# ipc-sim/IPC

Measured on NVIDIA H100. Metric: newton_iteration_ms_assembly_ccd, lower is better.
Workload: dtype f64

## Files before the change

ipc_b200/csrc/api.cu:

```cuda
#include "../../include/ipcgpu.h"
#include "context.h"
#include <algorithm>
#include <cmath>
#include <cstring>
#include <dlfcn.h>
#include <numeric>

using namespace ipcgpu;

#define CK(call)                                                                                  \
    do {                                                                                          \
        cudaError_t e_ = (call);                                                                  \
        if (e_ != cudaSuccess) {                                                                  \
            ctx->err = std::string(#call) + ": " + cudaGetErrorString(e_);                        \
            return IPCGPU_ERR_CUDA;                                                               \
        }                                                                                         \
    } while (0)
#define REQUIRE(cond, code, msg)                                                                  \
    do {                                                                                          \
        if (!(cond)) {                                                                            \
            ctx->err = (msg);                                                                     \
            return (code);                                                                        \
        }                                                                                         \
    } while (0)
// ... 16 lines not shown
bool nccl_load(std::string& err)
{
    if (g_nccl.h) return true;
    const char* names[] = { "libnccl.so.2", "libnccl.so" };
    for (const char* n : names) {
        g_nccl.h = dlopen(n, RTLD_NOW | RTLD_GLOBAL);
        if (g_nccl.h) break;
    }
    if (!g_nccl.h) {
        err = "dlopen(libnccl.so.2) failed";
        return false;
    }
    g_nccl.GetUniqueId = (int (*)(void*))dlsym(g_nccl.h, "ncclGetUniqueId");
    g_nccl.CommInitRank = (int (*)(void**, int, Id128, int))dlsym(g_nccl.h, "ncclCommInitRank");
    g_nccl.AllReduce = (int (*)(const void*, void*, size_t, int, int, void*, cudaStream_t))dlsym(g_nccl.h, "ncclAllReduce");
    g_nccl.AllGather = (int (*)(const void*, void*, size_t, int, void*, cudaStream_t))dlsym(g_nccl.h, "ncclAllGather");
    g_nccl.CommDestroy = (int (*)(void*))dlsym(g_nccl.h, "ncclCommDestroy");
    g_nccl.GetErrorString = (const char* (*)(int))dlsym(g_nccl.h, "ncclGetErrorString");
    if (!g_nccl.GetUniqueId || !g_nccl.CommInitRank || !g_nccl.AllReduce || !g_nccl.AllGather) {
        err = "NCCL symbols missing";
        return false;
    }
    return true;
}
constexpr int kNcclInt32 = 2;
constexpr int kNcclFloat64 = 8;
constexpr int kNcclUint64 = 5;
constexpr int kNcclSum = 0, kNcclMax = 2, kNcclMin = 3;
}

int nccl_min_u64(ipcgpu_ctx* ctx, unsigned long long* word)
{
    if (ctx->nranks <= 1) return IPCGPU_OK;
    cudaEvent_t pe = ctx->prof_begin(IPCGPU_STAGE_ALLREDUCE);
    int r = g_nccl.AllReduce(word, word, 1, kNcclUint64, kNcclMin, ctx->nccl_comm, ctx->stream);
    ctx->prof_end(pe);
    REQUIRE(r == 0, IPCGPU_ERR_NCCL, "ncclAllReduce(min step) failed");
    return IPCGPU_OK;
}

static int join_copy_stream(ipcgpu_ctx* ctx)
{
    if (!ctx->copy_pending) return IPCGPU_OK;
    CK(cudaEventRecord(ctx->ev_copy_join, ctx->copy));
    CK(cudaStreamWaitEvent(ctx->stream, ctx->ev_copy_join, 0));
    ctx->copy_pending = false;
    return IPCGPU_OK;
}

enum Chain { kSerial, kStepBound, kDerivative };

static int join_deriv(ipcgpu_ctx* ctx)
{
    if (!ctx->deriv_open) return IPCGPU_OK;
    ctx->deriv_open = false;
    CK(cudaEventRecord(ctx->ev_deriv_done, ctx->deriv));
    CK(cudaStreamWaitEvent(ctx->stream, ctx->ev_deriv_done, 0));
    return IPCGPU_OK;
}

static int enter(ipcgpu_ctx* ctx, Chain chain)
{
    if (chain == kStepBound) return IPCGPU_OK;
    if (chain == kSerial || ctx->nranks > 1 || ctx->profiling) return join_deriv(ctx);
    if (ctx->deriv_open) return IPCGPU_OK;
    CK(cudaEventRecord(ctx->ev_deriv_fork, ctx->stream));
    CK(cudaStreamWaitEvent(ctx->deriv, ctx->ev_deriv_fork, 0));
    ctx->deriv_open = true;
    return IPCGPU_OK;
}
#define ENTER(chain)                                                                              \
    do {                                                                                          \
        int re_ = enter(ctx, (chain));                                                            \
        if (re_) return re_;                                                                      \
    } while (0)

int fetch_iter_state(ipcgpu_ctx* ctx)
{
    {
        int rcj = join_copy_stream(ctx);
        if (rcj) return rcj;
    }
    CK(cudaMemcpyAsync(ctx->h_iter, ctx->iter.p, sizeof(IterState), cudaMemcpyDeviceToHost, ctx->stream));
    CK(cudaStreamSynchronize(ctx->stream));
    return IPCGPU_OK;
}
static int clear_flag(ipcgpu_ctx* ctx, int idx)
{
    CK(cudaMemsetAsync(&ctx->iter.p->flags[idx], 0, sizeof(int), ctx->stream));
    return IPCGPU_OK;
}

static int build_maps(ipcgpu_ctx* ctx)
{
    const int nT = ctx->nT, nV = ctx->nV;
    const std::vector<int>& T = ctx->h_T;
    ctx->t_begin = (int)((int64_t)nT * ctx->rank / ctx->nranks);
    ctx->t_end = (int)((int64_t)nT * (ctx->rank + 1) / ctx->nranks);
    std::vector<int64_t> cum(nV + 1, 0);
    for (size_t i = 0; i < (size_t)4 * nT; ++i) ++cum[T[i] + 1];
    for (int v = 0; v < nV; ++v) cum[v + 1] += cum[v];
    auto boundary = [&](int r) -> int {
        if (r <= 0) return 0;
        if (r >= ctx->nranks) return nV;
        const int64_t target = cum[nV] * r / ctx->nranks;
        return (int)(std::lower_bound(cum.begin(), cum.end(), target) - cum.begin());
// ... 1099 lines not shown
int ipcgpu_update_pattern(ipcgpu_ctx* ctx, int with_friction, int* changed, int64_t* nnz)
{
    REQUIRE(ctx->device_pattern, IPCGPU_ERR_STATE, "ipcgpu_enable_device_pattern first");
    REQUIRE(ctx->surface_ready, IPCGPU_ERR_STATE, "ipcgpu_set_surface first");
    REQUIRE(!with_friction || ctx->cw.fr_ready, IPCGPU_ERR_STATE, "with_friction: ipcgpu_friction_lag / ipcgpu_set_friction_data first");
    CK(cudaSetDevice(ctx->device));
    ENTER(kSerial);
    int rc = pattern_update(ctx, barrier_args(ctx, 1.0, 1.0, 0), with_friction != 0);
    if (rc) return rc;
    ctx->pat_pending = true;
    if (!changed && !nnz) return IPCGPU_OK;
    if ((rc = sync_pattern_mirror(ctx))) return rc;
    if (changed) *changed = ctx->pat_changed_host;
    if (nnz) *nnz = ctx->nnz;
    if (ctx->h_iter->flags[FLAG_PATTERN_CAPACITY]) {
        clear_flag(ctx, FLAG_PATTERN_CAPACITY);
        int only[8] = { 0 };
        only[FLAG_PATTERN_CAPACITY] = 1;
        return status_from_flags(ctx, only);
    }
    return IPCGPU_OK;
}

int ipcgpu_pattern_info(ipcgpu_ctx* ctx, int* changed, int64_t* nnz, uint64_t* version)
{
    REQUIRE(ctx->device_pattern, IPCGPU_ERR_STATE, "ipcgpu_enable_device_pattern first");
    CK(cudaSetDevice(ctx->device));
    ENTER(kSerial);
    int rc = sync_pattern_mirror(ctx);
    if (rc) return rc;
    if (changed) *changed = ctx->pat_changed_host;
    if (nnz) *nnz = ctx->nnz;
    if (version) *version = ctx->pat_seen_version;
    return IPCGPU_OK;
}

int ipcgpu_get_pattern(ipcgpu_ctx* ctx, int* ia, int* ja)
{
    REQUIRE(ctx->n_rows > 0, IPCGPU_ERR_STATE, "no pattern: ipcgpu_set_csr or ipcgpu_enable_device_pattern first");
    CK(cudaSetDevice(ctx->device));
    ENTER(kSerial);
    int rc = sync_pattern_mirror(ctx);
    if (rc) return rc;
    if (ia) CK(cudaMemcpyAsync(ia, ctx->ia.p, ((size_t)ctx->n_rows + 1) * sizeof(int), cudaMemcpyDeviceToHost, ctx->stream));
    if (ja) CK(cudaMemcpyAsync(ja, ctx->ja.p, (size_t)ctx->nnz * sizeof(int), cudaMemcpyDeviceToHost, ctx->stream));
    CK(cudaStreamSynchronize(ctx->stream));
    return IPCGPU_OK;
}

int ipcgpu_barrier_energy(ipcgpu_ctx* ctx, double dHat, double kappa, double* E)
{
    REQUIRE(ctx->surface_ready, IPCGPU_ERR_STATE, "ipcgpu_set_surface first");
    CK(cudaSetDevice(ctx->device));
    ENTER(kSerial);
    BarrierArgs p = barrier_args(ctx, dHat, kappa, 0);
    cudaEvent_t pe = ctx->prof_begin(IPCGPU_STAGE_BARRIER);
    barrier_energy(p, ctx->cw.bpartials.p, &ctx->iter.p->flags[FLAG_NONPOSITIVE_DISTANCE], ctx->stream);
    reduce_sum(ctx->cw.bpartials.p, barrier_energy_blocks(), kappa, ctx->scalar_out.p + 1, ctx->stream);
    ctx->prof_end(pe);
    ctx->launches += 2;
    if (ctx->nranks > 1 && E) {
        int r = g_nccl.AllReduce(ctx->scalar_out.p + 1, ctx->scalar_out.p + 1, 1, kNcclFloat64, kNcclSum, ctx->nccl_comm, ctx->stream);
        REQUIRE(r == 0, IPCGPU_ERR_NCCL, "ncclAllReduce(barrier energy) failed");
    }
    energy_store(ctx->iter.p, 1, ctx->scalar_out.p + 1, ctx->stream);
    ++ctx->launches;
    ctx->energy_local[1] = (ctx->nranks > 1 && !E);
    CK(cudaGetLastError());
    if (E) {
        int rc = fetch_iter_state(ctx);
        if (rc) return rc;
        *E = ctx->h_iter->energy[1];
        if (ctx->h_iter->flags[FLAG_NONPOSITIVE_DISTANCE]) {
            clear_flag(ctx, FLAG_NONPOSITIVE_DISTANCE);
            int only[8] = { 0 };
            only[FLAG_NONPOSITIVE_DISTANCE] = 1;
            return status_from_flags(ctx, only);
        }
    }
    return IPCGPU_OK;
}

int ipcgpu_barrier_gradient(ipcgpu_ctx* ctx, double dHat, double kappa, double* g_inout)
{
    REQUIRE(ctx->surface_ready, IPCGPU_ERR_STATE, "ipcgpu_set_surface first");
    CK(cudaSetDevice(ctx->device));
    ENTER(g_inout ? kSerial : kDerivative);
    if (g_inout) {
        if (ctx->rank == 0) CK(cudaMemcpyAsync(ctx->g.p, g_inout, (size_t)3 * ctx->nV * sizeof(double), cudaMemcpyHostToDevice, ctx->stream));
        else CK(cudaMemsetAsync(ctx->g.p, 0, (size_t)3 * ctx->nV * sizeof(double), ctx->stream));
    }
    cudaEvent_t pe = ctx->prof_begin(IPCGPU_STAGE_BARRIER);
    barrier_gradient(barrier_args(ctx, dHat, kappa, 0), ctx->g.p, ctx->deriv_stream());
    ctx->prof_end(pe);
    ++ctx->launches;
    CK(cudaGetLastError());
    if (g_inout && ctx->nranks > 1) {
        int rc = ipcgpu_allreduce_grad_hess(ctx, 1, 0);
        if (rc) return rc;
    }
    if (g_inout) {
        CK(cudaMemcpyAsync(g_inout, ctx->g.p, (size_t)3 * ctx->nV * sizeof(double), cudaMemcpyDeviceToHost, ctx->stream));
        CK(cudaStreamSynchronize(ctx->stream));
    }
    return IPCGPU_OK;
}

static int gradient_roundtrip_begin(ipcgpu_ctx* ctx, const double* g_in)
{
    if (ctx->rank == 0) CK(cudaMemcpyAsync(ctx->g.p, g_in, (size_t)3 * ctx->nV * sizeof(double), cudaMemcpyHostToDevice, ctx->stream));
    else CK(cudaMemsetAsync(ctx->g.p, 0, (size_t)3 * ctx->nV * sizeof(double), ctx->stream));
    return IPCGPU_OK;
}
static int gradient_roundtrip_end(ipcgpu_ctx* ctx, double* g_out)
{
    if (ctx->nranks > 1) {
        int rc = ipcgpu_allreduce_grad_hess(ctx, 1, 0);
        if (rc) return rc;
// ... 32 lines not shown
    CK(cudaSetDevice(ctx->device));
    ENTER(kSerial);
    ContactWork& w = ctx->cw;
    if (w.nC < 0) {
        int rc = contact_sync_counts(ctx);
        if (rc) return rc;
    }
    REQUIRE(n == w.nC && (input || n == 0), IPCGPU_ERR_ARG, "ipcgpu_constraint_jacobian_t: n must be the size of the active set on this context");
    REQUIRE(!(ctx->nranks > 1 && ctx->lists_local), IPCGPU_ERR_STATE, "per-constraint input needs the replicated sets (ipcgpu_set_contact_partition(0))");
    ALLOC(w.bval, (size_t)std::max(w.cap, 1));
    int rc = gradient_roundtrip_begin(ctx, g_inout);
    if (rc) return rc;
    if (n) CK(cudaMemcpyAsync(w.bval.p, input, (size_t)n * sizeof(double), cudaMemcpyHostToDevice, ctx->stream));
    BarrierArgs p = barrier_args(ctx, 1.0, 1.0, 0);
    p.cs = w.act.p; p.nC = w.counters.p + 0;
    constraint_jacobian_t(p, w.bval.p, coef, ctx->g.p, ctx->stream);
    ++ctx->launches;
    CK(cudaGetLastError());
    return gradient_roundtrip_end(ctx, g_inout);
}

int ipcgpu_para_ee_gradient(ipcgpu_ctx* ctx, double dHat, double kappa, double* g_inout)
{
    REQUIRE(ctx->surface_ready, IPCGPU_ERR_STATE, "ipcgpu_set_surface first");
    REQUIRE(g_inout != nullptr, IPCGPU_ERR_ARG, "null gradient");
    CK(cudaSetDevice(ctx->device));
    ENTER(kSerial);
    int rc = gradient_roundtrip_begin(ctx, g_inout);
    if (rc) return rc;
    para_gradient(barrier_args(ctx, dHat, kappa, 0), ctx->g.p, ctx->stream);
    ++ctx->launches;
    CK(cudaGetLastError());
    return gradient_roundtrip_end(ctx, g_inout);
}

int ipcgpu_barrier_hessian(ipcgpu_ctx* ctx, double dHat, double kappa, int projectDBC, double* a_inout)
{
    REQUIRE(ctx->surface_ready, IPCGPU_ERR_STATE, "ipcgpu_set_surface first");
    REQUIRE(ctx->nnz > 0, IPCGPU_ERR_STATE, "ipcgpu_set_csr first");
    CK(cudaSetDevice(ctx->device));
    ENTER(a_inout ? kSerial : kDerivative);
    int rc;
    if (a_inout && (rc = upload_values(ctx, a_inout))) return rc;
    ContactWork& w = ctx->cw;
    cudaEvent_t pe = ctx->prof_begin(IPCGPU_STAGE_BARRIER);
    const BarrierArgs bp = barrier_args(ctx, dHat, kappa, projectDBC);
    cudaStream_t st = ctx->deriv_stream();
    if (ctx->side && ctx->inputs_marked) {
        CK(cudaStreamWaitEvent(ctx->side, ctx->ev_inputs, 0));
        if (ctx->scatter_marked) CK(cudaStreamWaitEvent(ctx->side, ctx->ev_scatter, 0));
        barrier_hessian_build_project(bp, ctx->iter.p->flags, w.bHraw.p, w.brows.p, w.bpsd.p, w.counters.p + 12, w.cap, ctx->side);
        CK(cudaEventRecord(ctx->ev_join, ctx->side));
        CK(cudaStreamWaitEvent(st, ctx->ev_join, 0));
    }
    else barrier_hessian_build_project(bp, ctx->iter.p->flags, w.bHraw.p, w.brows.p, w.bpsd.p, w.counters.p + 12, w.cap, st);
    barrier_hessian_scatter(bp, ctx->a.p, ctx->iter.p->flags, w.bHraw.p, w.brows.p, w.bpsd.p, w.counters.p + 12, w.cap, st);
    if (ctx->side && ctx->ev_scatter) ctx->scatter_marked = (cudaEventRecord(ctx->ev_scatter, st) == cudaSuccess);
    ctx->prof_end(pe);
    ctx->launches += 3;
    CK(cudaGetLastError());
    if (a_inout) {
        if ((rc = download_values(ctx, a_inout))) return rc;
        if ((rc = fetch_iter_state(ctx))) return rc;
        if (ctx->h_iter->flags[FLAG_PATTERN] || ctx->h_iter->flags[FLAG_SET_CAPACITY]) {
            int only[8] = { 0 };
            only[FLAG_PATTERN] = ctx->h_iter->flags[FLAG_PATTERN];
            only[FLAG_SET_CAPACITY] = ctx->h_iter->flags[FLAG_SET_CAPACITY];
            clear_flag(ctx, FLAG_PATTERN);
            clear_flag(ctx, FLAG_SET_CAPACITY);
            return status_from_flags(ctx, only);
        }
    }
    return IPCGPU_OK;
}

int ipcgpu_set_prev_state(ipcgpu_ctx* ctx, const double* V_prev_soa)
{
    REQUIRE(ctx->nV > 0, IPCGPU_ERR_STATE, "ipcgpu_set_mesh first");
    CK(cudaSetDevice(ctx->device));
    ENTER(kSerial);
    ALLOC(ctx->Vprev, (size_t)3 * ctx->nV);
    if (V_prev_soa) CK(cudaMemcpyAsync(ctx->Vprev.p, V_prev_soa, (size_t)3 * ctx->nV * sizeof(double), cudaMemcpyHostToDevice, ctx->stream));
    else CK(cudaMemcpyAsync(ctx->Vprev.p, ctx->V.p, (size_t)3 * ctx->nV * sizeof(double), cudaMemcpyDeviceToDevice, ctx->stream));
    ctx->prev_set = true;
    return IPCGPU_OK;
}

static int friction_alloc(ipcgpu_ctx* ctx)
{
    ContactWork& w = ctx->cw;
    const size_t cap = (size_t)std::max(ctx->pair_capacity, 1);
    ALLOC(w.fr_cs, cap);
    ALLOC(w.fr_n, 1);
    ALLOC(w.fr_lambda, cap);
    ALLOC(w.fr_coord, cap);
    ALLOC(w.fr_basis, 6 * cap);
    ALLOC(w.fr_partials, (size_t)friction_energy_blocks() + 8);
    return IPCGPU_OK;
}

int ipcgpu_friction_lag(ipcgpu_ctx* ctx, double dHat, double kappa, int* n_pairs)
{
    REQUIRE(ctx->surface_ready, IPCGPU_ERR_STATE, "ipcgpu_set_surface first");
    CK(cudaSetDevice(ctx->device));
    ENTER(kSerial);
    int rc = friction_alloc(ctx);
    if (rc) return rc;
    ContactWork& w = ctx->cw;
    friction_lag(barrier_args(ctx, dHat, kappa, 0), w.fr_cs.p, w.fr_n.p, w.fr_lambda.p, w.fr_coord.p, w.fr_basis.p, ctx->pair_capacity,
        &ctx->iter.p->flags[FLAG_NONPOSITIVE_DISTANCE], ctx->stream);
    ++ctx->launches;
    CK(cudaGetLastError());
// ... 642 lines not shown
```

ipc_b200/csrc/barrier.cu:

```cuda
#include "pair_common.cuh"
#include "kernels.h"
#include <algorithm>

namespace ipcgpu {

template <typename PutH>
__device__ inline double pair_derivs(const PairStencil& s, const V3* x, double* g, bool want_h, PutH puth)
{
    if (s.kind == 3) {
        V3 r = 2.0 * (x[0] - x[1]);
        g[0] = r.x; g[1] = r.y; g[2] = r.z; g[3] = -r.x; g[4] = -r.y; g[5] = -r.z;
        if (want_h)
            for (int i = 0; i < 6; ++i)
                for (int j = 0; j < 6; ++j) puth(i, j, (i == j) ? 2.0 : ((i % 3 == j % 3) ? -2.0 : 0.0));
        return norm2(x[0] - x[1]);
    }
    Diff D;
    if (s.kind == 0) plane_dist(x[0] - x[1], x[2] - x[1], x[3] - x[1], D);
    else if (s.kind == 1) plane_dist(x[2] - x[0], x[1] - x[0], x[3] - x[2], D);
    else line_dist(x[0] - x[1], x[2] - x[1], D);
    diff_to_vertices(D, s.kind, s.nv, true, want_h, [&](int i, double v) { g[i] = v; }, puth);
    return D.val;
}

// ... 450 lines not shown
        int o = -1;
        const int vi = rows[bi], vj = rows[bj];
        if (vi >= 0 && vj >= 0 && vi <= vj && !(vi == vj && bi != bj) && owns_row(p, vi) && !proj_dbc(p.dbc, vi, p.projectDBC) && !proj_dbc(p.dbc, vj, p.projectDBC)) {
            const int c0 = (vi == vj) ? r : 0;
            o = csr_find(p.ia, p.ja, p.base, 3 * vi + r, 3 * vj + c0);
            if (o < 0) o = -2;
            else o -= c0;
        }
        sOff[wib][t] = o;
    }
    __syncwarp();
#pragma unroll
    for (int kk = 0; kk < 5; ++kk) {
        const int e = lane + 32 * kk;
        if (e < 144) {
            const int i = e / 12, j = e % 12;
            const int bi = i / 3, r = i % 3, bj = j / 3, q = j % 3;
            const int o = sOff[wib][(bi * 4 + bj) * 3 + r];
            if (o == -2) atomicExch(err, 1);
            else if (o != -1) {
                if (rows[bi] == rows[bj] && q < r) continue;
                double v = 0.0;
                if (raw) v = H0[i * 12 + j];
                else {
#pragma unroll
                    for (int ka = 0; ka < 3; ++ka) {
                        const double qa = helmert(ka, bi);
#pragma unroll
                        for (int kb = 0; kb < 3; ++kb) v += (qa * helmert(kb, bj)) * H0[(3 * ka + r) * 9 + 3 * kb + q];
                    }
                }
                atomicAdd(a + o + q, v);
            }
        }
    }
    __syncwarp();
    }
}

void barrier_energy(const BarrierArgs& p, double* partials, int* bad, cudaStream_t st)
{
    k_barrier_energy<<<kBarrierEnergyBlocks, 256, 0, st>>>(p, partials, bad);
}
int barrier_energy_blocks() { return kBarrierEnergyBlocks; }
void barrier_gradient(const BarrierArgs& p, double* g, cudaStream_t st)
{
    k_barrier_gradient<<<kSMs * 4, 128, 0, st>>>(p, g);
}
void evaluate_constraints(const BarrierArgs& p, double* val, cudaStream_t st) { k_evaluate_constraints<<<kSMs * 2, 256, 0, st>>>(p, val); }
void constraint_jacobian_t(const BarrierArgs& p, const double* input, double coef, double* g, cudaStream_t st) { k_constraint_jacobian_t<<<kSMs * 4, 128, 0, st>>>(p, input, coef, g); }
void para_gradient(const BarrierArgs& p, double* g, cudaStream_t st) { k_para_gradient<<<kSMs, 128, 0, st>>>(p, g); }
void barrier_hessian_build_project(const BarrierArgs& p, int* flags, double* Hraw, int* rows, int* psd, int* n_owned, int capacity, cudaStream_t st)
{
    cudaMemsetAsync(n_owned, 0, sizeof(int), st);
    k_barrier_hessian_build<<<kSMs * 8, 64, 0, st>>>(p, Hraw, rows, n_owned, capacity, flags);
    k_barrier_hessian_project<<<kSMs * 4, 32 * kProjWarps, 0, st>>>(n_owned, capacity, Hraw, psd);
}
void barrier_hessian_scatter(const BarrierArgs& p, double* a, int* flags, const double* Hraw, const int* rows, const int* psd, const int* n_owned, int capacity, cudaStream_t st)
{
    k_barrier_hessian_scatter<<<kSMs * 4, 32 * kScatWarps, 0, st>>>(p, n_owned, capacity, Hraw, rows, psd, a, flags + FLAG_PATTERN);
}

}
```

ipc_b200/csrc/ccd.cu:

```cuda
#include "broadphase.cuh"
#include "context.h"
#include "../../include/ipcgpu.h"
#include <cub/cub.cuh>

namespace ipcgpu {

__global__ void __launch_bounds__(256) k_ref_ranges(SurfArgs s, const double* __restrict__ dir, const IterState* __restrict__ st, int* __restrict__ vmin, int* __restrict__ vmax)
{
    const int i = blockIdx.x * blockDim.x + threadIdx.x;
    if (i >= s.nSV) return;
    const double alpha = st->alpha_grid, inv_h = st->ref_inv_h;
    const int v = s.SVI[i];
#pragma unroll
    for (int c = 0; c < 3; ++c) {
        const double x = s.V[(size_t)c * s.nV + v];
        const double xt = x + alpha * dir[3 * (size_t)v + c];
        const int a = (int)floor((x - st->ref_lo[c]) * inv_h), b = (int)floor((xt - st->ref_lo[c]) * inv_h);
        vmin[3 * (size_t)v + c] = min(a, b);
        vmax[3 * (size_t)v + c] = max(a, b);
    }
}

__global__ void __launch_bounds__(256) k_swept_bounds(SurfArgs s, const double* __restrict__ dir, const IterState* __restrict__ st, unsigned long long* __restrict__ bounds)
{
// ... 1528 lines not shown
    const IterState& h = *ctx->h_iter;
    w.last_survivors = (unsigned)h.ccd_stats[0];
    w.last_warnings = (int)h.ccd_stats[1];
    w.last_deferred = h.ccd_stats[2];
    w.last_longest_cycles = h.ccd_stats[3];
    w.last_total_cycles = h.ccd_stats[4];
    w.last_boxes_thread = h.ccd_stats[5];
    w.last_boxes_warp = h.ccd_stats[6];
    w.last_candidates = h.ccd_stats[7];
    if (alpha_out) std::memcpy(alpha_out, &h.step_ord, sizeof(double));
    return 0;
}

int ccd_build_swept(ipcgpu_ctx* ctx, double h)
{
    CcdWork& w = ctx->ccd;
    cudaStream_t st = ctx->stream;
    const SurfArgs s = surf_args(ctx);
    IterState* ist = ctx->iter.p;
    if (!ctx->dir_valid) {
        ctx->err = "no search direction: pass p (or call ipcgpu_set_search_dir first)";
        return IPCGPU_ERR_STATE;
    }
    cudaEvent_t pe = ctx->prof_begin(IPCGPU_STAGE_CCD_BROAD);
    k_swept_alpha<<<1, 32, 0, st>>>(ist, ctx->pSize_dev.p, h, w.bounds.p);
    k_swept_bounds<<<std::min(nblk(std::max(s.nV, s.nSV), 256), kSMs * 4), 256, 0, st>>>(s, ctx->dir.p, ist, w.bounds.p);
    k_refgrid_params<<<1, 32, 0, st>>>(ist, w.bounds.p, h, w.cells.p);
    ctx->launches += 3;
    const int nPrim = s.nSF + s.nSE + s.nSV;
    if (s.nSV > 0) {
        k_ref_ranges<<<nblk(s.nSV, 256), 256, 0, st>>>(s, ctx->dir.p, ist, w.vmin.p, w.vmax.p);
        k_swept_extent<<<std::min(nblk(nPrim, 256), kSMs * 4), 256, 0, st>>>(s, w.vmin.p, w.vmax.p, w.cells.p);
        k_swept_cells<<<1, 32, 0, st>>>(w.cells.p);
        const size_t nTab = (size_t)3 * kGridCells + 1;
        zero_words(w.sw_cnt.p, nTab, st);
        k_swept_count<<<nblk(nPrim, 256), 256, 0, st>>>(s, w.vmin.p, w.vmax.p, w.cells.p, w.sw_cnt.p);
        size_t bytes = w.sw_tmp.n;
        CKD(cub::DeviceScan::ExclusiveSum(w.sw_tmp.p, bytes, w.sw_cnt.p, w.sw_off.p, (int)nTab, st));
        k_swept_scatter<<<nblk(nPrim, 256), 256, 0, st>>>(s, w.vmin.p, w.vmax.p, w.cells.p, w.sw_cnt.p, w.sw_off.p, w.sw_keys.p, w.sw_ent.p);
        ctx->launches += 7;
    }
    ctx->prof_end(pe);
    CKD(cudaGetLastError());
    w.swept_ready = true;
    return 0;
}

int ccd_full(ipcgpu_ctx* ctx, double tol, const double* err_vf, const double* err_ee)
{
    CcdWork& w = ctx->ccd;
    cudaStream_t st = ctx->stream;
    const SurfArgs s = surf_args(ctx);
    cudaEvent_t pe = ctx->prof_begin(IPCGPU_STAGE_CCD_BROAD);
    CKD(cudaMemsetAsync(w.ncand.p, 0, 2 * sizeof(unsigned long long), st));
    CKD(cudaMemsetAsync(w.counters.p + 14, 0, sizeof(int), st));
    SweptArgs a{ s, ctx->dir.p, ctx->iter.p, w.vmin.p, w.vmax.p, w.cells.p, w.sw_keys.p, w.sw_ent.p, w.sw_off.p, 0, 0,
        CandOut{ w.cand.p, w.ncand.p, (unsigned long long)ctx->ccd_capacity, w.counters.p + 14 } };
    if (s.nSF > 0 && s.nSV > 0) {
        a.lo = (int)((long long)s.nSV * ctx->rank / ctx->nranks);
        a.hi = (int)((long long)s.nSV * (ctx->rank + 1) / ctx->nranks);
        k_swept_pairs_pt<<<kSMs * 8, 32 * kSweptWarps, 0, st>>>(a);
        ++ctx->launches;
    }
    if (s.nSE > 1) {
        a.lo = (int)((long long)s.nSE * ctx->rank / ctx->nranks);
        a.hi = (int)((long long)s.nSE * (ctx->rank + 1) / ctx->nranks);
        k_swept_pairs_ee<<<kSMs * 8, 32 * kSweptWarps, 0, st>>>(a);
        ++ctx->launches;
    }
    ctx->prof_end(pe);
    return ccd_narrow(ctx, w.cand.p, nullptr, w.ncand.p, (unsigned long long)ctx->ccd_capacity, 0, tol, err_vf, err_ee, 3, w.counters.p + 14);
}
```

ipc_b200/csrc/constraint.cu:

```cuda
#include "broadphase.cuh"
#include "context.h"
#include "../../include/ipcgpu.h"
#include <cub/cub.cuh>

namespace ipcgpu {

DEV void grow(Box& b, V3 x)
{
    b.lo[0] = fmin(b.lo[0], x.x); b.hi[0] = fmax(b.hi[0], x.x);
    b.lo[1] = fmin(b.lo[1], x.y); b.hi[1] = fmax(b.hi[1], x.y);
    b.lo[2] = fmin(b.lo[2], x.z); b.hi[2] = fmax(b.hi[2], x.z);
}
DEV Box empty_box()
{
    Box b;
    for (int a = 0; a < 3; ++a) { b.lo[a] = 1e300; b.hi[a] = -1e300; }
    return b;
}

__global__ void __launch_bounds__(256) k_boxes(SurfArgs s, int prim, Box* __restrict__ boxes, unsigned long long* __restrict__ bounds)
{
    const int n = prim == 0 ? s.nSV : (prim == 1 ? s.nSE : s.nSF);
    const int i = blockIdx.x * blockDim.x + threadIdx.x;
    Box b = empty_box();
// ... 810 lines not shown
    cudaStream_t st = ctx->stream;
    const SurfArgs s = surf_args(ctx);
    k_bounds_init<<<1, 32, 0, st>>>(w.bounds.p);
    if (with_vertex_boxes && s.nSV > 0) k_boxes<<<nblk(s.nSV, 256), 256, 0, st>>>(s, 0, w.vbox.p, w.bounds.p);
    if (s.nSE > 0) k_boxes<<<nblk(s.nSE, 256), 256, 0, st>>>(s, 1, w.ebox.p, w.bounds.p);
    if (s.nSF > 0) k_boxes<<<nblk(s.nSF, 256), 256, 0, st>>>(s, 2, w.tbox.p, w.bounds.p);
    k_grid_params<<<1, 32, 0, st>>>(w.bounds.p, radius, w.axis_bits, w.grid.p, ctx->iter.p);
    ctx->launches += 5;
    return build_grids(ctx, s.nSF, s.nSE, (with_vertex_boxes && pairs_mode() != 0) ? s.nSV : 0);
}

void contact_pack_lists(ipcgpu_ctx* ctx)
{
    ContactWork& w = ctx->cw;
    k_pack_lists<<<kSMs, 256, 0, ctx->stream>>>(w.act.p, w.para.p, w.para_e.p, w.counters.p, w.xcap, w.xsend.p, &ctx->iter.p->flags[FLAG_EXCHANGE_CAPACITY]);
    ++ctx->launches;
}
void contact_unpack_lists(ipcgpu_ctx* ctx)
{
    ContactWork& w = ctx->cw;
    k_unpack_lists<<<kSMs, 256, 0, ctx->stream>>>(w.xrecv.p, ctx->nranks, w.xcap, w.xstride, w.gact.p, w.gpara.p, w.gpara_e.p, w.cap, w.counters.p + 10,
        &ctx->iter.p->flags[FLAG_EXCHANGE_CAPACITY]);
    ++ctx->launches;
}

int contact_sync_counts(ipcgpu_ctx* ctx)
{
    ContactWork& w = ctx->cw;
    int* h = reinterpret_cast<int*>(ctx->h_scalar);
    CKC(cudaMemcpyAsync(h, w.counters.p, 8 * sizeof(int), cudaMemcpyDeviceToHost, ctx->stream));
    CKC(cudaStreamSynchronize(ctx->stream));
    if (h[4]) {
        ctx->err = "constraint-set capacity exceeded (raise it with ipcgpu_set_pair_capacity)";
        return IPCGPU_ERR_CAPACITY;
    }
    w.nC = h[0];
    w.nP = h[2];
    w.nK = w.want_cand ? h[3] : 0;
    return 0;
}

int contact_constraint_set(ipcgpu_ctx* ctx, double dHat, int wantCand, int* nC, int* nPara, int* nCand)
{
    ContactWork& w = ctx->cw;
    cudaStream_t st = ctx->stream;
    const SurfArgs s = surf_args(ctx);
    const double radius = sqrt(dHat);
    cudaEvent_t pe = ctx->prof_begin(IPCGPU_STAGE_HASH);
    int rc;
    if ((rc = boxes_and_grid(ctx, radius, pairs_mode() != 0))) return rc;
    ctx->prof_end(pe);

    pe = ctx->prof_begin(IPCGPU_STAGE_CONSTRAINT_SET);
    CKC(cudaMemsetAsync(w.counters.p, 0, 16 * sizeof(int), st));
    CsOut out;
    out.act = w.act.p; out.nAct = w.counters.p + 0; out.capAct = w.cap;
    out.dup = w.dup.p; out.nDup = w.counters.p + 1; out.capDup = w.cap;
    out.para = w.para.p; out.para_e = w.para_e.p; out.nPara = w.counters.p + 2; out.capPara = w.cap;
    out.cand = w.cand.p; out.nCand = w.counters.p + 3; out.capCand = 4 * w.cap;
    out.overflow = w.counters.p + 4;
    const SortedGrid tg = tri_grid(ctx), eg = edge_grid(ctx);
    int v0 = 0, v1 = s.nSV, e0 = 0, e1 = s.nSE;
    if (ctx->partition_contact && ctx->nranks > 1) {
        v0 = (int)((long long)s.nSV * ctx->rank / ctx->nranks); v1 = (int)((long long)s.nSV * (ctx->rank + 1) / ctx->nranks);
        e0 = (int)((long long)s.nSE * ctx->rank / ctx->nranks); e1 = (int)((long long)s.nSE * (ctx->rank + 1) / ctx->nranks);
    }
    unsigned* nPairs = reinterpret_cast<unsigned*>(w.counters.p + 8);
    PairOut ppt{ w.bp_pairs.p, nPairs, (unsigned)w.bp_cap, w.counters.p + 4 }, pee{ w.bp_pairs.p + w.bp_cap, nPairs + 1, (unsigned)w.bp_cap, w.counters.p + 4 };
    if (v1 > v0 && s.nSF > 0) {
        if (pairs_mode() == 0 || w.built_vertices != s.nSV) k_pairs_pt<<<nblk(v1 - v0, 8 * kPairQueriesPerWarp), 256, 0, st>>>(s, w.grid.p, tg, dHat, radius, v0, v1, ppt);
        else cell_pairs_pt(w.grid.p, vertex_grid(ctx), tg, s, radius, s.nSF + s.nSE + v0, s.nSF + s.nSE + v1, ppt, st);
        k_classify_pt<<<kSMs * 8, 128, 0, st>>>(s, ppt.pairs, ppt.n, ppt.cap, dHat, wantCand, out);
        ctx->launches += 2;
    }
    if (e1 > e0 && s.nSE > 1) {
        if (pairs_mode() == 0) k_pairs_ee<<<nblk(e1 - e0, 8 * kPairQueriesPerWarp), 256, 0, st>>>(w.grid.p, eg, w.ebox.p, dHat, radius, s.nSF + e0, s.nSF + e1, pee);
        else cell_pairs_ee(w.grid.p, eg, s, radius, s.nSF + e0, s.nSF + e1, pee, st);
        k_classify_ee<<<kSMs * 8, 128, 0, st>>>(s, pee.pairs, pee.n, pee.cap, dHat, wantCand, out);
        ctx->launches += 2;
    }
    const bool hashed_merge = ctx->nV < (1 << 21) - 2;
    if (hashed_merge) {
        CKC(cudaMemsetAsync(w.skey.p, 0xff, (size_t)w.dup_tab * sizeof(unsigned long long), st));
        CKC(cudaMemsetAsync(w.sidx.p, 0, (size_t)w.dup_tab * sizeof(int), st));
        k_dup_insert<<<kSMs * 2, 256, 0, st>>>(w.counters.p + 1, w.cap, w.dup.p, w.skey.p, w.sidx.p, w.dup_tab - 1, w.counters.p + 4);
        k_dup_emit<<<nblk(w.dup_tab, 256), 256, 0, st>>>(w.dup_tab, w.skey.p, w.sidx.p, w.act.p, w.counters.p + 0, w.cap, w.counters.p + 4);
        ctx->launches += 2;
    }
    w.want_cand = wantCand != 0;
    w.nC = w.nP = w.nK = -1;
    const bool need_host = !hashed_merge || ctx->canonical_order || nC || nPara || nCand;
    if (need_host) {
        int* h = reinterpret_cast<int*>(ctx->h_scalar);
        if (!hashed_merge) {
            CKC(cudaMemcpyAsync(h, w.counters.p, 8 * sizeof(int), cudaMemcpyDeviceToHost, st));
            CKC(cudaStreamSynchronize(st));
            const int nDup = std::min(h[1], w.cap);
            if (nDup > 0) {
                if ((rc = sort_lex(ctx, w.dup.p, nullptr, nDup, w.tmp4.p, nullptr))) return rc;
                k_merge_dups<<<nblk(nDup, 256), 256, 0, st>>>(nDup, w.dup.p, w.act.p, w.counters.p + 0, w.cap, w.counters.p + 4);
                ++ctx->launches;
            }
        }
        if ((rc = contact_sync_counts(ctx))) return rc;
        if (ctx->canonical_order) {
            if ((rc = sort_lex(ctx, w.act.p, nullptr, w.nC, w.tmp4.p, nullptr))) return rc;
            if ((rc = sort_lex(ctx, w.para.p, w.para_e.p, w.nP, w.tmp4.p, w.tmp2.p))) return rc;
            if (wantCand && (rc = sort_int2(ctx, w.cand.p, w.nK, w.tmp2.p))) return rc;
        }
    }
    k_publish_counts<<<1, 32, 0, st>>>(w.counters.p, wantCand, ctx->iter.p);
    ++ctx->launches;
    ctx->prof_end(pe);
    if (nC) *nC = w.nC;
    if (nPara) *nPara = w.nP;
    if (nCand) *nCand = w.nK;
    return 0;
}
```

ipc_b200/csrc/context.h:

```cpp
#pragma once
#include "kernels.h"
#include "broadphase_types.h"
#include <cuda_runtime.h>
#include <cstdint>
#include <cstring>
#include <string>
#include <vector>

namespace ipcgpu {

template <typename T>
struct DevBuf {
    T* p = nullptr;
    size_t n = 0;
    ~DevBuf() { release(); }
    void release()
    {
        if (p) cudaFree(p);
        p = nullptr;
        n = 0;
    }
    bool reserve(size_t count)
    {
        if (count <= n) return true;
// ... 36 lines not shown
    DevBuf<int> brows, bpsd;
    int xcap = 0;
    size_t xstride = 0;
    DevBuf<int4> xsend, xrecv, gact, gpara;
    DevBuf<int2> gpara_e;
    bool lists_global = false;
    DevBuf<int4> fr_cs;
    DevBuf<int> fr_n;
    DevBuf<double> fr_lambda, fr_basis, fr_partials;
    DevBuf<double2> fr_coord;
    int fr_host_n = -1;
    bool fr_ready = false;
};

struct CcdWork {
    DevBuf<int> vmin, vmax, counters;
    DevBuf<int2> cand;
    DevBuf<unsigned> surv, surv2;
    bool wide_level_set = false;
    DevBuf<unsigned char> scratch;
    DevBuf<unsigned long long> ncand, bounds;
    DevBuf<SweptCells> cells;
    DevBuf<unsigned> sw_keys;
    DevBuf<uint4> sw_ent;
    DevBuf<int> sw_cnt, sw_off;
    DevBuf<unsigned char> sw_tmp;
    bool swept_ready = false;
    unsigned last_survivors = 0;
    unsigned long long last_deferred = 0, last_longest_cycles = 0, last_total_cycles = 0;
    int last_warnings = 0;
    unsigned long long last_candidates = 0, last_boxes_thread = 0, last_boxes_warp = 0;
};

struct PatternWork {
    DevBuf<int> mptr, mnbr;
    DevBuf<int> row_cnt, row_off;
    DevBuf<int> bucket;
    DevBuf<int> ucnt, uoff;
    DevBuf<int> prev_ptr, prev_nbr;
    DevBuf<unsigned char> scan_tmp;
    size_t scan_bytes = 0;
    long long mesh_pairs = 0, mesh_nnz = 0, nnz_cap = 0, key_cap = 0;
    uint64_t requested_cap = 0;
};

}

struct ipcgpu_ctx {
    int device = 0;
    cudaStream_t stream = nullptr;
    cudaStream_t deriv = nullptr;
    cudaEvent_t ev_deriv_fork = nullptr, ev_deriv_done = nullptr;
    bool deriv_open = false, deriv_copied = false;
    int prio_low = 0, prio_high = 0;
    cudaStream_t deriv_stream() const { return deriv_open ? deriv : stream; }
    cudaStream_t side = nullptr;
    cudaStream_t copy = nullptr;
    cudaEvent_t ev_copy_fork = nullptr, ev_copy_join = nullptr;
    bool copy_pending = false;
    cudaEvent_t ev_inputs = nullptr, ev_join = nullptr, ev_scatter = nullptr;
    bool scatter_marked = false;
    bool inputs_marked = false;
    void mark_inputs()
    {
        if (ev_inputs) inputs_marked = (cudaEventRecord(ev_inputs, stream) == cudaSuccess);
    }
    std::string err;
    uint64_t launches = 0;

    int rank = 0, nranks = 1;
    void* nccl_comm = nullptr;
    int v_begin = 0, v_end = 0, n_list = 0;
    ipcgpu::DevBuf<int> tet_list;
    long long a_begin = 0, a_end = 0;

    ipcgpu::DevBuf<ipcgpu::IterState> iter;
    ipcgpu::IterState* h_iter = nullptr;
    double pSize = 0.0;
    bool dir_valid = false, pSize_surface = false;
    bool energy_local[4] = { false, false, false, false };
    bool a_all_dirty = false;
    bool checks_local = false;
    std::vector<int> h_ia;

    int nV = 0, nT = 0, energy = 0;
    int t_begin = 0, t_end = 0;
    ipcgpu::DevBuf<double> V, Vsaved, Vrest, Ainv, vol, mu, lam, mass, Vprev, xtilde;
    bool prev_set = false, xtilde_set = false;
    ipcgpu::DevBuf<int> T;
    ipcgpu::DevBuf<uint8_t> dbc;
    bool has_mass = false, has_dbc = false, state_saved = false;
    std::vector<int> h_T;

    int nSV = 0, nSE = 0, nSF = 0;
    int nVdof = 0x7fffffff;
    int ee_as_vf = 1;
    ipcgpu::DevBuf<int> SVI, SE, SF, vCoDim;
    bool has_codim = false, surface_ready = false;
    int pair_capacity = 1 << 20;
    int exchange_capacity = 1 << 16;
    bool canonical_order = true;
    bool partition_contact = false, lists_local = false;
    ipcgpu::ContactWork cw;
    ipcgpu::CcdWork ccd;
    size_t ccd_capacity = (size_t)1 << 23;
    std::vector<int> h_SVI;
// ... 74 lines not shown
```

ipc_b200/csrc/kernels.h:

```cpp
#pragma once
#include <cuda_runtime.h>
#include <cstdint>

namespace ipcgpu {

struct IterState {
    unsigned long long step_ord;
    unsigned long long inv_ord;
    unsigned long long ccd_ord;
    unsigned long long cand_range[2];
    unsigned long long n_full_cand;
    double max_t;
    double alpha_grid;
    double ref_lo[3], ref_inv_h;
    double alpha_stage[4];
    double energy[4];
    int ref_count[3];
    int n_set[3];
    int flags[8];
    int grid_axis_cells;
    int pad_;
    int checks[2];
    unsigned long long ccd_stats[8];
    long long pat_nnz;
// ... 57 lines not shown
__device__ __forceinline__ bool obstacle_vertex(const SurfArgs& s, int v) { return v >= s.nVdof; }

struct BarrierArgs {
    int nV;
    const double* V;
    const double* Vrest;
    const uint8_t* dbc;
    const int* SE;
    const int4* cs; const int* nC;
    const int4* para; const int2* para_e; const int* nP;
    int rank, nranks, share;
    int row_lo, row_hi;
    double dHat, kappa;
    int projectDBC;
    const int* ia; const int* ja; int base;
    int nVdof;
};

void barrier_energy(const BarrierArgs& p, double* partials, int* bad, cudaStream_t st);
int barrier_energy_blocks();
void barrier_gradient(const BarrierArgs& p, double* g, cudaStream_t st);
void evaluate_constraints(const BarrierArgs& p, double* val, cudaStream_t st);
void constraint_jacobian_t(const BarrierArgs& p, const double* input, double coef, double* g, cudaStream_t st);
void para_gradient(const BarrierArgs& p, double* g, cudaStream_t st);
void barrier_hessian_build_project(const BarrierArgs& p, int* flags, double* Hraw, int* rows, int* psd, int* n_owned, int capacity, cudaStream_t st);
void barrier_hessian_scatter(const BarrierArgs& p, double* a, int* flags, const double* Hraw, const int* rows, const int* psd, const int* n_owned, int capacity, cudaStream_t st);
struct FrictionArgs {
    int nV;
    const double* V;
    const double* Vt;
    const uint8_t* dbc;
    const int4* cs; const int* n;
    const double* lambda;
    const double2* coord;
    const double* basis;
    double eps2, coef;
    int projectDBC;
    const int* ia; const int* ja; int base;
    int rank, nranks;
    int row_lo, row_hi;
};
void friction_lag(const BarrierArgs& p, int4* cs_out, int* n_out, double* lambda, double2* coord, double* basis, int capacity, int* bad, cudaStream_t st);
void friction_energy(const FrictionArgs& p, double* partials, cudaStream_t st);
int friction_energy_blocks();
void friction_gradient(const FrictionArgs& p, double* g, cudaStream_t st);
void friction_hessian(const FrictionArgs& p, double* a, int* err, cudaStream_t st);
void zero_csr_rows(const int* ia, int base, int row0, int row1, double* a, cudaStream_t st);
void reduce_sum(const double* partials, int n, double scale, double* out, cudaStream_t st);

void step_forward(int nV, const double* x0_soa, const double* p_interleaved, double alpha, double* x_soa, cudaStream_t st);
int inertia_energy_blocks(int nV);
void inertia_energy(int v0, int v1, int nV, const double* x_soa, const double* xtilde_soa, const double* mass, double* partials, cudaStream_t st);
void inertia_gradient(int nV, const double* x_soa, const double* xtilde_soa, const double* mass, const uint8_t* dbc, int projectDBC, double* g, cudaStream_t st);
void zero_words(void* p, size_t n_words, cudaStream_t st);

}
```

ipc_b200/csrc/misc.cu:

```cuda
#include "common.cuh"
#include "kernels.h"
#include <algorithm>

namespace ipcgpu {

__global__ void __launch_bounds__(256) k_step_forward(int nV, const double* __restrict__ x0, const double* __restrict__ p, double alpha, double* __restrict__ x)
{
    const int v = blockIdx.x * blockDim.x + threadIdx.x;
    if (v >= nV) return;
#pragma unroll
    for (int c = 0; c < 3; ++c) x[(size_t)c * nV + v] = x0[(size_t)c * nV + v] + alpha * p[3 * (size_t)v + c];
}

void step_forward(int nV, const double* x0, const double* p, double alpha, double* x, cudaStream_t st)
{
    if (nV > 0) k_step_forward<<<(nV + 255) / 256, 256, 0, st>>>(nV, x0, p, alpha, x);
}

__global__ void __launch_bounds__(256) k_inertia_energy(int v0, int v1, int nV, const double* __restrict__ x, const double* __restrict__ xt, const double* __restrict__ mass,
    double* __restrict__ partials)
{
    const int v = v0 + blockIdx.x * blockDim.x + threadIdx.x;
    double e = 0.0;
    if (v < v1) {
        double s = 0.0;
#pragma unroll
        for (int c = 0; c < 3; ++c) {
            const double d = x[(size_t)c * nV + v] - xt[(size_t)c * nV + v];
            s += d * d;
        }
        e = s * mass[v] / 2.0;
    }
    __shared__ double sm[8];
    const double w = warp_sum(e);
    if ((threadIdx.x & 31) == 0) sm[threadIdx.x >> 5] = w;
    __syncthreads();
    if (threadIdx.x == 0) {
        double s = 0.0;
#pragma unroll
        for (int i = 0; i < 8; ++i) s += sm[i];
        partials[blockIdx.x] = s;
    }
}
__global__ void __launch_bounds__(256) k_inertia_gradient(int nV, const double* __restrict__ x, const double* __restrict__ xt, const double* __restrict__ mass,
    const uint8_t* __restrict__ dbc, int projectDBC, double* __restrict__ g)
{
    const int v = blockIdx.x * blockDim.x + threadIdx.x;
    if (v >= nV) return;
    if (dbc && (dbc[v] == 1 || (dbc[v] == 2 && projectDBC))) return;
    const double m = mass[v];
#pragma unroll
    for (int c = 0; c < 3; ++c) g[3 * (size_t)v + c] += m * (x[(size_t)c * nV + v] - xt[(size_t)c * nV + v]);
}
int inertia_energy_blocks(int nV) { return (nV + 255) / 256; }
void inertia_energy(int v0, int v1, int nV, const double* x, const double* xt, const double* mass, double* partials, cudaStream_t st)
{
    if (v1 > v0) k_inertia_energy<<<(v1 - v0 + 255) / 256, 256, 0, st>>>(v0, v1, nV, x, xt, mass, partials);
}
void inertia_gradient(int nV, const double* x, const double* xt, const double* mass, const uint8_t* dbc, int projectDBC, double* g, cudaStream_t st)
{
    if (nV > 0) k_inertia_gradient<<<(nV + 255) / 256, 256, 0, st>>>(nV, x, xt, mass, dbc, projectDBC, g);
}

__global__ void __launch_bounds__(256) k_zero_words(size_t n, unsigned* __restrict__ p)
{
    for (size_t i = (size_t)blockIdx.x * blockDim.x + threadIdx.x; i < n; i += (size_t)gridDim.x * blockDim.x) p[i] = 0u;
}
void zero_words(void* p, size_t n_words, cudaStream_t st)
{
    if (n_words) k_zero_words<<<(unsigned)std::min<size_t>((n_words + 255) / 256, (size_t)kSMs * 16), 256, 0, st>>>(n_words, static_cast<unsigned*>(p));
}

}
```

Baseline: 2.937.

## Run barrier energy on side stream and replace memsets with fill kernels

When barrier energy is requested without a host readback, it now takes the derivative chain and runs on the side stream, so it overlaps with elastic and derivative work. A side_open flag makes sure the side stream is joined back into the main stream. Several cudaMemsetAsync calls are replaced by a small fill kernel that takes a fill value, which keeps graph capture to kernel nodes only. The new cross-stream dependency adds some risk of ordering mistakes and adds a few extra launches.

```diff
diff --git a/ipc_b200/csrc/api.cu b/ipc_b200/csrc/api.cu
--- a/ipc_b200/csrc/api.cu
+++ b/ipc_b200/csrc/api.cu
@@ -92,6 +92,11 @@
 
 static int join_deriv(ipcgpu_ctx* ctx)
 {
+    if (ctx->side_open) {
+        ctx->side_open = false;
+        CK(cudaEventRecord(ctx->ev_join, ctx->side));
+        CK(cudaStreamWaitEvent(ctx->stream, ctx->ev_join, 0));
+    }
     if (!ctx->deriv_open) return IPCGPU_OK;
     ctx->deriv_open = false;
     CK(cudaEventRecord(ctx->ev_deriv_done, ctx->deriv));
@@ -1297,18 +1302,24 @@
 {
     REQUIRE(ctx->surface_ready, IPCGPU_ERR_STATE, "ipcgpu_set_surface first");
     CK(cudaSetDevice(ctx->device));
-    ENTER(kSerial);
+    ENTER(E ? kSerial : kDerivative);
     BarrierArgs p = barrier_args(ctx, dHat, kappa, 0);
+    cudaStream_t st = ctx->deriv_stream();
+    if (ctx->deriv_open && ctx->side && ctx->inputs_marked) {
+        CK(cudaStreamWaitEvent(ctx->side, ctx->ev_inputs, 0));
+        st = ctx->side;
+        ctx->side_open = true;
+    }
     cudaEvent_t pe = ctx->prof_begin(IPCGPU_STAGE_BARRIER);
-    barrier_energy(p, ctx->cw.bpartials.p, &ctx->iter.p->flags[FLAG_NONPOSITIVE_DISTANCE], ctx->stream);
-    reduce_sum(ctx->cw.bpartials.p, barrier_energy_blocks(), kappa, ctx->scalar_out.p + 1, ctx->stream);
+    barrier_energy(p, ctx->cw.bpartials.p, &ctx->iter.p->flags[FLAG_NONPOSITIVE_DISTANCE], st);
+    reduce_sum(ctx->cw.bpartials.p, barrier_energy_blocks(), kappa, ctx->scalar_out.p + 1, st);
     ctx->prof_end(pe);
     ctx->launches += 2;
     if (ctx->nranks > 1 && E) {
         int r = g_nccl.AllReduce(ctx->scalar_out.p + 1, ctx->scalar_out.p + 1, 1, kNcclFloat64, kNcclSum, ctx->nccl_comm, ctx->stream);
         REQUIRE(r == 0, IPCGPU_ERR_NCCL, "ncclAllReduce(barrier energy) failed");
     }
-    energy_store(ctx->iter.p, 1, ctx->scalar_out.p + 1, ctx->stream);
+    energy_store(ctx->iter.p, 1, ctx->scalar_out.p + 1, st);
     ++ctx->launches;
     ctx->energy_local[1] = (ctx->nranks > 1 && !E);
     CK(cudaGetLastError());
@@ -1447,12 +1458,13 @@
         barrier_hessian_build_project(bp, ctx->iter.p->flags, w.bHraw.p, w.brows.p, w.bpsd.p, w.counters.p + 12, w.cap, ctx->side);
         CK(cudaEventRecord(ctx->ev_join, ctx->side));
         CK(cudaStreamWaitEvent(st, ctx->ev_join, 0));
+        ctx->side_open = false;
     }
     else barrier_hessian_build_project(bp, ctx->iter.p->flags, w.bHraw.p, w.brows.p, w.bpsd.p, w.counters.p + 12, w.cap, st);
     barrier_hessian_scatter(bp, ctx->a.p, ctx->iter.p->flags, w.bHraw.p, w.brows.p, w.bpsd.p, w.counters.p + 12, w.cap, st);
     if (ctx->side && ctx->ev_scatter) ctx->scatter_marked = (cudaEventRecord(ctx->ev_scatter, st) == cudaSuccess);
     ctx->prof_end(pe);
-    ctx->launches += 3;
+    ctx->launches += 4;
     CK(cudaGetLastError());
     if (a_inout) {
         if ((rc = download_values(ctx, a_inout))) return rc;
diff --git a/ipc_b200/csrc/barrier.cu b/ipc_b200/csrc/barrier.cu
--- a/ipc_b200/csrc/barrier.cu
+++ b/ipc_b200/csrc/barrier.cu
@@ -526,7 +526,7 @@
 void para_gradient(const BarrierArgs& p, double* g, cudaStream_t st) { k_para_gradient<<<kSMs, 128, 0, st>>>(p, g); }
 void barrier_hessian_build_project(const BarrierArgs& p, int* flags, double* Hraw, int* rows, int* psd, int* n_owned, int capacity, cudaStream_t st)
 {
-    cudaMemsetAsync(n_owned, 0, sizeof(int), st);
+    zero_words(n_owned, 1, st);
     k_barrier_hessian_build<<<kSMs * 8, 64, 0, st>>>(p, Hraw, rows, n_owned, capacity, flags);
     k_barrier_hessian_project<<<kSMs * 4, 32 * kProjWarps, 0, st>>>(n_owned, capacity, Hraw, psd);
 }
diff --git a/ipc_b200/csrc/ccd.cu b/ipc_b200/csrc/ccd.cu
--- a/ipc_b200/csrc/ccd.cu
+++ b/ipc_b200/csrc/ccd.cu
@@ -1604,8 +1604,9 @@
     cudaStream_t st = ctx->stream;
     const SurfArgs s = surf_args(ctx);
     cudaEvent_t pe = ctx->prof_begin(IPCGPU_STAGE_CCD_BROAD);
-    CKD(cudaMemsetAsync(w.ncand.p, 0, 2 * sizeof(unsigned long long), st));
-    CKD(cudaMemsetAsync(w.counters.p + 14, 0, sizeof(int), st));
+    zero_words(w.ncand.p, 4, st);
+    zero_words(w.counters.p + 14, 1, st);
+    ctx->launches += 2;
     SweptArgs a{ s, ctx->dir.p, ctx->iter.p, w.vmin.p, w.vmax.p, w.cells.p, w.sw_keys.p, w.sw_ent.p, w.sw_off.p, 0, 0,
         CandOut{ w.cand.p, w.ncand.p, (unsigned long long)ctx->ccd_capacity, w.counters.p + 14 } };
     if (s.nSF > 0 && s.nSV > 0) {
diff --git a/ipc_b200/csrc/constraint.cu b/ipc_b200/csrc/constraint.cu
--- a/ipc_b200/csrc/constraint.cu
+++ b/ipc_b200/csrc/constraint.cu
@@ -886,7 +886,8 @@
     ctx->prof_end(pe);
 
     pe = ctx->prof_begin(IPCGPU_STAGE_CONSTRAINT_SET);
-    CKC(cudaMemsetAsync(w.counters.p, 0, 16 * sizeof(int), st));
+    zero_words(w.counters.p, 16, st);
+    ++ctx->launches;
     CsOut out;
     out.act = w.act.p; out.nAct = w.counters.p + 0; out.capAct = w.cap;
     out.dup = w.dup.p; out.nDup = w.counters.p + 1; out.capDup = w.cap;
@@ -915,11 +916,11 @@
     }
     const bool hashed_merge = ctx->nV < (1 << 21) - 2;
     if (hashed_merge) {
-        CKC(cudaMemsetAsync(w.skey.p, 0xff, (size_t)w.dup_tab * sizeof(unsigned long long), st));
-        CKC(cudaMemsetAsync(w.sidx.p, 0, (size_t)w.dup_tab * sizeof(int), st));
+        zero_words(w.skey.p, (size_t)w.dup_tab * 2, st, 0xffffffffu);
+        zero_words(w.sidx.p, w.dup_tab, st);
         k_dup_insert<<<kSMs * 2, 256, 0, st>>>(w.counters.p + 1, w.cap, w.dup.p, w.skey.p, w.sidx.p, w.dup_tab - 1, w.counters.p + 4);
         k_dup_emit<<<nblk(w.dup_tab, 256), 256, 0, st>>>(w.dup_tab, w.skey.p, w.sidx.p, w.act.p, w.counters.p + 0, w.cap, w.counters.p + 4);
-        ctx->launches += 2;
+        ctx->launches += 4;
     }
     w.want_cand = wantCand != 0;
     w.nC = w.nP = w.nK = -1;
diff --git a/ipc_b200/csrc/context.h b/ipc_b200/csrc/context.h
--- a/ipc_b200/csrc/context.h
+++ b/ipc_b200/csrc/context.h
@@ -112,6 +112,7 @@
     cudaStream_t deriv = nullptr;
     cudaEvent_t ev_deriv_fork = nullptr, ev_deriv_done = nullptr;
     bool deriv_open = false, deriv_copied = false;
+    bool side_open = false;
     int prio_low = 0, prio_high = 0;
     cudaStream_t deriv_stream() const { return deriv_open ? deriv : stream; }
     cudaStream_t side = nullptr;
diff --git a/ipc_b200/csrc/kernels.h b/ipc_b200/csrc/kernels.h
--- a/ipc_b200/csrc/kernels.h
+++ b/ipc_b200/csrc/kernels.h
@@ -133,6 +133,6 @@
 int inertia_energy_blocks(int nV);
 void inertia_energy(int v0, int v1, int nV, const double* x_soa, const double* xtilde_soa, const double* mass, double* partials, cudaStream_t st);
 void inertia_gradient(int nV, const double* x_soa, const double* xtilde_soa, const double* mass, const uint8_t* dbc, int projectDBC, double* g, cudaStream_t st);
-void zero_words(void* p, size_t n_words, cudaStream_t st);
+void zero_words(void* p, size_t n_words, cudaStream_t st, unsigned fill = 0u);
 
 }
diff --git a/ipc_b200/csrc/misc.cu b/ipc_b200/csrc/misc.cu
--- a/ipc_b200/csrc/misc.cu
+++ b/ipc_b200/csrc/misc.cu
@@ -62,13 +62,13 @@
     if (nV > 0) k_inertia_gradient<<<(nV + 255) / 256, 256, 0, st>>>(nV, x, xt, mass, dbc, projectDBC, g);
 }
 
-__global__ void __launch_bounds__(256) k_zero_words(size_t n, unsigned* __restrict__ p)
+__global__ void __launch_bounds__(256) k_zero_words(size_t n, unsigned fill, unsigned* __restrict__ p)
 {
-    for (size_t i = (size_t)blockIdx.x * blockDim.x + threadIdx.x; i < n; i += (size_t)gridDim.x * blockDim.x) p[i] = 0u;
+    for (size_t i = (size_t)blockIdx.x * blockDim.x + threadIdx.x; i < n; i += (size_t)gridDim.x * blockDim.x) p[i] = fill;
 }
-void zero_words(void* p, size_t n_words, cudaStream_t st)
+void zero_words(void* p, size_t n_words, cudaStream_t st, unsigned fill)
 {
-    if (n_words) k_zero_words<<<(unsigned)std::min<size_t>((n_words + 255) / 256, (size_t)kSMs * 16), 256, 0, st>>>(n_words, static_cast<unsigned*>(p));
+    if (n_words) k_zero_words<<<(unsigned)std::min<size_t>((n_words + 255) / 256, (size_t)kSMs * 16), 256, 0, st>>>(n_words, fill, static_cast<unsigned*>(p));
 }
 
 }
diff --git a/profiles/iteration_timeline.py b/profiles/iteration_timeline.py
--- /dev/null
+++ b/profiles/iteration_timeline.py
@@ -0,0 +1,150 @@
+import argparse
+import json
+import os
+import subprocess
+import sys
+
+import numpy as np
+
+ROOT = os.path.dirname(os.path.dirname(os.path.abspath(__file__)))
+sys.path.insert(0, ROOT)
+
+import bench
+from ipc_b200 import lib as L
+
+DT2 = 0.025 ** 2
+
+
+class Args:
+    tets, res, scene = 1_000_000, 10, "c5"
+
+
+def gpu_info():
+    try:
+        q = subprocess.check_output(["nvidia-smi", "--query-gpu=name,clocks.sm,clocks.max.sm,power.limit", "--format=csv,noheader"], text=True)
+        return q.strip().splitlines()[0]
+    except Exception as e:
+        return f"nvidia-smi unavailable: {e}"
+
+
+def iterations(kernels, n):
+    groups = {}
+    for k in kernels:
+        groups.setdefault(k.get("args", {}).get("correlation"), []).append(k)
+    full = [g for g in groups.values() if any("k_publish_counts" in k["name"] for k in g) and any("k_elastic_grad_hess" in k["name"] for k in g)]
+    if len(full) == n:
+        return sorted(full, key=lambda g: min(k["ts"] for k in g)), "correlation"
+    ks = sorted(kernels, key=lambda k: k["ts"])
+    out, end = [], -1e30
+    for k in ks:
+        if k["ts"] > end + 15.0:
+            out.append([])
+        out[-1].append(k)
+        end = max(end, k["ts"] + k["dur"])
+    return [g for g in out if any("k_publish_counts" in k["name"] for k in g)], "gaps"
+
+
+def first(g, name):
+    ks = [k for k in g if name in k["name"]]
+    return min(ks, key=lambda k: k["ts"]) if ks else None
+
+
+def row(g):
+    t0 = min(k["ts"] for k in g if k["cat"] == "kernel")
+    pub, el, sc, pt = first(g, "k_publish_counts"), first(g, "k_elastic_grad_hess"), first(g, "k_swept_scatter"), first(g, "k_swept_pairs_pt")
+    return {"front": pub["ts"] + pub["dur"] - t0, "elastic_start": el["ts"] - t0,
+            "swept_gap": pt["ts"] - (sc["ts"] + sc["dur"]) if sc and pt else None,
+            "ti_kernel": sum(k["dur"] for k in g if "k_ti_" in k["name"]),
+            "span": max(k["ts"] + k["dur"] for k in g if k["cat"] == "kernel") - t0,
+            "copy_end": max((k["ts"] + k["dur"] for k in g if k["cat"] == "gpu_memcpy" and "DtoH" in k["name"]), default=t0) - t0 or None,
+            "kernels": sum(1 for k in g if k["cat"] == "kernel")}
+
+
+def main():
+    ap = argparse.ArgumentParser()
+    ap.add_argument("out_dir")
+    ap.add_argument("--reps", type=int, default=20)
+    ap.add_argument("--download", action="store_true", help="bench.py's end-to-end graph: the gradient and CSR values copied to the host")
+    args = ap.parse_args()
+    import torch
+    from torch.profiler import ProfilerActivity, profile
+
+    os.makedirs(args.out_dir, exist_ok=True)
+    m, info = bench.build_scene(Args())
+    dHat, h = info["dHat"], m.avgEdgeLen / 3
+    ctx = L.Context(0)
+    ctx.set_mesh(m.V_rest_soa, m.T_soa, m.restTriInv, m.vol, m.mu, m.lam, m.mass, m.dbc, m.energy)
+    ctx.set_surface(m.SVI, m.SFEdges, m.SF_soa, m.vCoDim)
+    ctx.set_state(m.V_soa)
+    evf, eee = L.Context.ti_error(m.V_soa, m.nV, None)
+    mm, pa, pe, _ = ctx.constraint_set(dHat, 1)
+    ia, ja = m.csr_pattern(1, extra_pairs=bench.contact_pattern_pairs(m, mm, pa, pe))
+    ctx.set_csr(ia, ja, 1)
+    ctx.set_contact_partition(1)
+    ctx.set_canonical_order(0)
+    ctx.set_search_dir(info["p"])
+    hV, hp = L.PinnedArray(3 * m.nV), L.PinnedArray(3 * m.nV)
+    hV.array[:] = m.V_soa
+    hp.array[:] = info["p"]
+    hg, ha = L.PinnedArray(3 * m.nV), L.PinnedArray(ja.size)
+
+    def enqueue():
+        ctx.constraint_set(dHat, 1, fetch=False, sizes=False)
+        ctx.barrier_energy(dHat, bench.KAPPA, want=False)
+        ctx.elastic_energy_grad_hess(DT2, 1, 1, 1, None, None)
+        ctx.barrier_gradient(dHat, bench.KAPPA, None)
+        ctx.barrier_hessian(dHat, bench.KAPPA, 1, None)
+        ctx.allreduce_grad_hess(1, 0)
+        if args.download:
+            ctx.download_range_async(L.BUF_GRADIENT, 0, hg.array)
+            ctx.download_range_async(L.BUF_CSR_VALUES, 0, ha.array)
+        ctx.step_bound_set(1.0)
+        ctx.inversion_step(None, 0.2, None)
+        ctx.ccd_partial(None, bench.TI_TOL, evf, eee, None)
+        ctx.hash_build_swept(None, None, h)
+        ctx.ccd_full(bench.TI_TOL, evf, eee, None)
+
+    for _ in range(3):
+        enqueue()
+        assert ctx.fetch_iteration().status == 0
+    ctx.capture_begin()
+    enqueue()
+    graph = ctx.capture_end()
+
+    def replay():
+        if args.download:
+            ctx.set_state(hV.array)
+            ctx.set_search_dir(hp.array)
+        ctx.graph_launch(graph)
+        assert ctx.fetch_iteration().status == 0
+
+    for _ in range(5):
+        replay()
+    out = {"gpu": gpu_info(), "scene": f"C5, {m.nT} tets, {m.nV} vertices", "reps": args.reps, "graph": "end to end" if args.download else "device resident"}
+    torch.cuda.init()
+    with profile(activities=[ProfilerActivity.CUDA]) as prof:
+        for _ in range(args.reps):
+            replay()
+    trace = os.path.join(args.out_dir, "trace.pt.trace.json")
+    prof.export_chrome_trace(trace)
+    with open(trace) as f:
+        ev = json.load(f)
+    kernels = [e for e in (ev["traceEvents"] if isinstance(ev, dict) else ev) if e.get("ph") == "X" and e.get("cat") in ("kernel", "gpu_memcpy")]
+    its, how = iterations(kernels, args.reps)
+    rows = [row(g) for g in its]
+    out["split_by"] = how
+    out["iterations"] = len(rows)
+    out["median_us"] = {k: float(np.median([r[k] for r in rows if r[k] is not None])) for k in ("front", "elastic_start", "swept_gap", "ti_kernel", "span", "copy_end")
+                       if any(r[k] is not None for r in rows)}
+    out["gpu_after"] = gpu_info()
+    with open(os.path.join(args.out_dir, "timeline.json"), "w") as f:
+        json.dump({**out, "rows": rows}, f, indent=1)
+    print(json.dumps(out))
+    ctx.graph_destroy(graph)
+    for a in (hV, hp, hg, ha):
+        a.free()
+    ctx.close()
+
+
+if __name__ == "__main__":
+    main()
```

Result: no change. 2.916, median of 6 (-0.7%).
